# pxl-th/SLAM.jl

Hardware: AMD Instinct MI355X
Metric: frames/sec KITTI-05 stereo @1k kpts; local-BA ms/iter for 50-KF window (higher is better)
Workload: dtype f64

## Files before the change

### slam.jl_amd/csrc/common.hpp

```cpp
#pragma once
#include <hip/hip_runtime.h>
#include <cstdint>
#include <cstdio>
#include <cstring>
#include <string>
#include <vector>
#include <mutex>
#include "../../include/slamhip.h"

#define SLAM_MAX_LEVELS 8

struct slam_ctx {
    int device = 0;
    hipStream_t stream = nullptr;
    int cus = 0;
    int dev_cus = 0;
    bool arch_ok = false;
    bool xwg_ok = false;
    int pool_class = 99;
    std::string err;
    void *scratch = nullptr; size_t scratch_bytes = 0;
    void *scratch2 = nullptr; size_t scratch2_bytes = 0;
    void *pinned = nullptr; size_t pinned_bytes = 0;
    hipEvent_t wait_event = nullptr;
    hipStream_t stream2 = nullptr;
    hipEvent_t fork_ev = nullptr, join_ev = nullptr;
    bool prof_on = false;
    struct ProfSpan { int id; hipEvent_t a, b; };
    std::vector<ProfSpan> prof_pending;
    std::vector<hipEvent_t> prof_pool;
    std::vector<std::string> prof_names;
    std::vector<double> prof_ms;
    std::vector<long long> prof_cnt;
};

extern "C" hipStream_t ctx_aux_stream(slam_ctx *c);
extern "C" void ctx_probe_device(slam_ctx *c);

struct ProfScope {
    slam_ctx *c; int idx;
    ProfScope(slam_ctx *ctx, const char *name);
    ~ProfScope();
};

struct LevelView {
    double *L, *Iy, *Ix, *Iyy, *Ixx, *Iyx;
    int H, W, P;
};
struct PyrView {
    LevelView lv[SLAM_MAX_LEVELS];
    int levels;
};

struct slam_pyr {
    int device = 0;
    int levels = 0;
    int H[SLAM_MAX_LEVELS], W[SLAM_MAX_LEVELS];
    int P[SLAM_MAX_LEVELS];
    int64_t off[SLAM_MAX_LEVELS + 1];
    struct Alloc { double *base = nullptr; double *ck = nullptr; double *tot = nullptr; const void **srctab = nullptr; double *xc = nullptr; int *xf = nullptr; int xseg = 0; int refs = 0; std::mutex graph_mu; };
    Alloc *alloc = nullptr;
    size_t zstride = 0;
    int batch_index = 0, batch_size = 1;
    bool tol_planes = false;
    bool target_only = false;
    double *planes = nullptr;
    double *tmp = nullptr;
    double *ck = nullptr;
    double *norm = nullptr;
    double norm_sigma = -1.0;
    struct Graph { int mode; double sigma; int S; size_t ckmin; int src_kind; hipGraphExec_t exec; };
    std::vector<Graph> graphs;
    bool graph_failed = false;
    PyrView view;
    double *plane(int p, int l) const { return planes + (int64_t)p * off[levels] + off[l]; }
};

struct slam_kpset {
    int device = 0, S = 0, cap = 0;
    char *base = nullptr;
    double *yx = nullptr;
    double *oyx = nullptr;
    double *syx = nullptr;
    double *xyz = nullptr;
    double *kyx = nullptr;
    uint8_t *haskf = nullptr;
    double *fyx = nullptr;
    int *fkf = nullptr;
    int *kfcount = nullptr;
    int64_t *id = nullptr;
    uint8_t *is3d = nullptr, *stereo = nullptr, *st = nullptr;
    int *count = nullptr;
    int *work = nullptr;
    int *ntot = nullptr;
    int64_t *next_id = nullptr;
    double *par = nullptr, *par_host = nullptr;
    hipEvent_t par_ev[8] = {};
    int par_slot = 0;
};
int kpset_stage_params(slam_ctx *ctx, slam_kpset *ks, const double *host, size_t n, const double **dev_out);

extern thread_local std::string g_slam_err;

hipError_t slam_stream_wait(hipStream_t s);

int slam_fail(slam_ctx *ctx, int code, const char *fmt, ...);
int slam_scratch(slam_ctx *ctx, size_t bytes, void **out);
int slam_scratch2(slam_ctx *ctx, size_t bytes, void **out);
int slam_pinned(slam_ctx *ctx, size_t bytes, void **out);

#define HIP_TRY(ctx, expr)                                                                  \
    do {                                                                                    \
        hipError_t _e = (expr);                                                             \
        if (_e != hipSuccess)                                                               \
            return slam_fail((ctx), SLAM_ERR_HIP, "%s: %s (%s:%d)", #expr, hipGetErrorString(_e), __FILE__, __LINE__); \
    } while (0)

#define ARG_TRY(ctx, cond)                                                                  \
    do {                                                                                    \
        if (!(cond)) return slam_fail((ctx), SLAM_ERR_ARG, "argument check failed: %s (%s:%d)", #cond, __FILE__, __LINE__); \
    } while (0)

#define SLAM_PYR_TARGET_ONLY 16
#define SLAM_PYR_CHAIN 32
#define SLAM_PYR_FLAGS (SLAM_PYR_TARGET_ONLY | SLAM_PYR_CHAIN)
struct IIRCoef {
    double a1, a2, a3, scale, M[9], inv1masum , inv1mbsum ;
};
IIRCoef slam_iir_coef(double sigma);
int slam_gaussian_taps(double sigma, double *w);

struct Cam { double fx, fy, cx, cy; };
struct PnPArgs {
    Cam cam; const double *px; const double *pts; int n;
    double X0[6]; int iters_fast, iterations; double depth_eps, repr_eps;
    uint8_t *outl; double *result;
};
int pnp_launch_device(slam_ctx *ctx, int S, const PnPArgs *args_dev);

int kpset_build_worklist(slam_ctx *ctx, slam_kpset *ks);
int kpset_compact(slam_ctx *ctx, slam_kpset *ks, int mode, const uint8_t *flags_dev);
int slam_detect_device(slam_ctx *ctx, const double *img_dev, int H, int W, int pitch, const double *cur_yx, int n_cur,
                       int max_points, int radius, int grid_rows, int grid_cols, int cell_size,
// ... 2 lines not shown
```

### slam.jl_amd/csrc/pyramid.hip

```cpp
#include "common.hpp"
#include <cmath>
#include <cstdlib>
#include <mutex>
#include <tuple>
#include <utility>

#define LINE_THREADS 64

struct PlaneSet {
    double *p[4];
    const double *nrm[4];
    int coef[4];
    int fill0[4];
    const double *sq[4];
    int n;
    size_t zs;
};
#define PS_PICK(ps, f, pl) ((pl) == 0 ? (ps).f[0] : (pl) == 1 ? (ps).f[1] : (pl) == 2 ? (ps).f[2] : (ps).f[3])
__device__ __forceinline__ double *ps_plane(const PlaneSet &ps, int pl) { return PS_PICK(ps, p, pl) + (size_t)blockIdx.z * ps.zs; }
__device__ __forceinline__ const double *ps_nrm(const PlaneSet &ps, int pl) { return PS_PICK(ps, nrm, pl); }
__device__ __forceinline__ int ps_coef(const PlaneSet &ps, int pl) { return PS_PICK(ps, coef, pl); }
__device__ __forceinline__ bool ps_fill0(const PlaneSet &ps, int pl) { return PS_PICK(ps, fill0, pl) != 0; }
__device__ __forceinline__ const double *ps_sq(const PlaneSet &ps, int pl) { const double *q = PS_PICK(ps, sq, pl); return q ? q + (size_t)blockIdx.z * ps.zs : nullptr; }

// ... 1019 lines not shown
        const int x0 = cb * CF_W, wc = W - x0 < CF_W ? W - x0 : CF_W;
#pragma unroll
        for (int sub = 0; sub < 4; sub++)
#pragma unroll
            for (int r = 0; r < 4; r++) { const v2d t2 = {raw[sub][2 * r], raw[sub][2 * r + 1]}; *(ldsv2 *)(Cb + (8 * r + cg) * CF_LS + sub * 16 + 2 * rp) = t2; }
        cf_load_block(plane, P, cb + 1 < ncb ? x0 + CF_W : x0, r0, voff, raw);
        double acc = 0.0;
        if (SEG && w == 0 && seg > 0) {
            if (lane == 0) while (__hip_atomic_load(xf_in, __ATOMIC_RELAXED, __HIP_MEMORY_SCOPE_AGENT) <= cb) __builtin_amdgcn_s_sleep(2);
            __builtin_amdgcn_fence(__ATOMIC_ACQUIRE, "wavefront"); __builtin_amdgcn_wave_barrier();
            if (lane < CF_W && x0 + lane < W) acc = __hip_atomic_load(xc_in + x0 + lane, __ATOMIC_RELAXED, __HIP_MEMORY_SCOPE_AGENT);
        }
        if (w > 0) {
            while (flag_ld(&s_ready[w - 1]) <= cb) __builtin_amdgcn_s_sleep(1);
            __builtin_amdgcn_fence(__ATOMIC_ACQUIRE, "workgroup", "local");
            if (lane < CF_W) acc = carry_in[(cb & 1) * CF_W + lane];
            __builtin_amdgcn_fence(__ATOMIC_RELEASE, "workgroup", "local");
            if (lane == 0) flag_st(&s_done[w], cb + 1);
        }
        __builtin_amdgcn_fence(__ATOMIC_RELEASE, "wavefront"); __builtin_amdgcn_wave_barrier();
        if (lane < CF_W) {
            ldsd *c = Cb + lane * CF_LS;
            if (hr == 64 && (SEG ? r0 > 0 : w > 0)) {
#pragma unroll
                for (int half = 0; half < 2; half++) {
                    double v[32];
#pragma unroll
                    for (int j = 0; j < 16; j++) { const v2d q = *(const ldsv2 *)(c + 32 * half + 2 * j); v[2 * j] = q.x; v[2 * j + 1] = q.y; }
#pragma unroll
                    for (int e = 0; e < 32; e++) { acc = acc + v[e]; v[e] = acc; }
#pragma unroll
                    for (int j = 0; j < 16; j++) { const v2d t2 = {v[2 * j], v[2 * j + 1]}; *(ldsv2 *)(c + 32 * half + 2 * j) = t2; }
                }
            } else {
                for (int e = 0; e < hr; e++) { acc = (r0 + e == 0) ? c[e] : acc + c[e]; c[e] = acc; }
            }
        }
        if (w + 1 < nwh) {
            while (flag_ld(&s_done[w + 1]) + 2 <= cb) __builtin_amdgcn_s_sleep(1);
            if (lane < CF_W) carry_out[(cb & 1) * CF_W + lane] = acc;
            __builtin_amdgcn_fence(__ATOMIC_RELEASE, "workgroup", "local");
            if (lane == 0) flag_st(&s_ready[w], cb + 1);
        }
        else if (SEG && seg + 1 < nseg) {
            if (lane < CF_W && x0 + lane < W) __hip_atomic_store(xc_out + x0 + lane, acc, __ATOMIC_RELAXED, __HIP_MEMORY_SCOPE_AGENT);
            asm volatile("s_waitcnt vmcnt(0)" ::: "memory");
            if (lane == 0) __hip_atomic_store(xf_out, cb + 1, __ATOMIC_RELAXED, __HIP_MEMORY_SCOPE_AGENT);
        }
        __builtin_amdgcn_fence(__ATOMIC_RELEASE, "wavefront"); __builtin_amdgcn_wave_barrier();
        if (lane < hr) {
            ldsd *c = Cb + lane;
            if (wc == CF_W && cb > 0) {
                double v[CF_W];
#pragma unroll
                for (int j = 0; j < CF_W; j++) v[j] = c[j * CF_LS];
#pragma unroll
                for (int j = 0; j < CF_W; j++) { rcarry = rcarry + v[j]; v[j] = rcarry; }
#pragma unroll
                for (int j = 0; j < CF_W; j++) c[j * CF_LS] = v[j];
            } else {
                for (int j = 0; j < wc; j++) { rcarry = (cb == 0 && j == 0) ? c[j * CF_LS] : rcarry + c[j * CF_LS]; c[j * CF_LS] = rcarry; }
            }
        }
        __builtin_amdgcn_fence(__ATOMIC_RELEASE, "wavefront"); __builtin_amdgcn_wave_barrier();
#pragma unroll
        for (int sub = 0; sub < 4; sub++) {
            const int rb = r0 + sub * 16;
            if (rb < H) {
#pragma unroll
                for (int r = 0; r < 4; r++) {
                    const int col = x0 + 8 * r + cg, row = rb + 2 * rp;
                    const v2d q = *(const ldsv2 *)(Cb + (8 * r + cg) * CF_LS + sub * 16 + 2 * rp);
                    double *g = plane + ((size_t)(x0 + 8 * r) * P + rb) + voff;
                    if (col < W) {
                        if (row + 1 < H) __builtin_nontemporal_store(q, (v2d *)g);
                        else if (row < H) g[0] = q.x;
                    }
                }
            }
        }
        __builtin_amdgcn_fence(__ATOMIC_RELEASE, "wavefront"); __builtin_amdgcn_wave_barrier();
    }
    if (SEG && w == 0 && seg > 0 && lane == 0) __hip_atomic_store(xf_in, 0, __ATOMIC_RELAXED, __HIP_MEMORY_SCOPE_AGENT);
}

#define PAR_T 1024
#define PAR_SLMAX 16
#define PAR_G 8
struct SegPow { double P[2][PAR_G][9]; double Plast[2][9]; };

__device__ __forceinline__ void mv3(const double *P, double &a, double &b, double &c, double za, double zb, double zc)
{
    const double n1 = __builtin_fma(P[0], a, __builtin_fma(P[1], b, __builtin_fma(P[2], c, za)));
    const double n2 = __builtin_fma(P[3], a, __builtin_fma(P[4], b, __builtin_fma(P[5], c, zb)));
    const double n3 = __builtin_fma(P[6], a, __builtin_fma(P[7], b, __builtin_fma(P[8], c, zc)));
    a = n1; b = n2; c = n3;
}

template <int ZG, int ZL, int GG, int GL, int ZN, int GN, class Slot>
__device__ __forceinline__ void fold_entry(const SegPow &sp, int cs, double (*Z)[ZN], double (*GT)[GN],
                                           int l, int k, bool has, Slot slot, double s0a, double s0b, double s0c,
                                           double &ea, double &eb, double &ec)
{
    const int q = k % PAR_G, grp = k / PAR_G;
    const double *P1 = sp.P[cs][0], *P8 = sp.P[cs][PAR_G - 1];
    double a = 0.0, b = 0.0, c = 0.0;
    if (has) for (int i = 0; i < q; i++) { const int s = slot(grp * PAR_G + i); mv3(P1, a, b, c, Z[0][s * ZG + l * ZL], Z[1][s * ZG + l * ZL], Z[2][s * ZG + l * ZL]); }
    if (has && q == PAR_G - 1) {
        double ta = a, tb = b, tc = c; const int s = slot(k);
        mv3(P1, ta, tb, tc, Z[0][s * ZG + l * ZL], Z[1][s * ZG + l * ZL], Z[2][s * ZG + l * ZL]);
        GT[0][grp * GG + l * GL] = ta; GT[1][grp * GG + l * GL] = tb; GT[2][grp * GG + l * GL] = tc;
    }
    __syncthreads();
    double Sa = s0a, Sb = s0b, Sc = s0c;
    if (has) {
        for (int h = 0; h < grp; h++) mv3(P8, Sa, Sb, Sc, GT[0][h * GG + l * GL], GT[1][h * GG + l * GL], GT[2][h * GG + l * GL]);
        if (q > 0) mv3(sp.P[cs][q - 1], Sa, Sb, Sc, 0.0, 0.0, 0.0);
    }
    ea = Sa + a; eb = Sb + b; ec = Sc + c;
}

template <bool COLS, int T = PAR_T, int LPW = 8>
__global__ __launch_bounds__(T) void k_iir_seg(PlaneSet ps, const double *src0, int H, int W, int P, IIRPair cf, SegPow sp, int SL, int cum_mask)
{
    if (src0) src0 += (size_t)blockIdx.z * ps.zs;
    constexpr int NSEG = T / LPW, ZN = T + 8, GN = T / PAR_G + 16;
    constexpr int ZG = COLS ? 1 : LPW, ZL = COLS ? NSEG + 1 : 1, GG = COLS ? 1 : LPW, GL = COLS ? NSEG / PAR_G + 2 : 1;
    __shared__ double Z[3][ZN];
    __shared__ double GT[3][GN];
    __shared__ double Fin[3][LPW];
    const int t = threadIdx.x, l = COLS ? t / NSEG : t % LPW, g = COLS ? t % NSEG : t / LPW, pl = blockIdx.y;
    const int nlines = COLS ? W : H, n = COLS ? H : W;
    const int line = blockIdx.x * LPW + l;
    const bool valid = line < nlines;
    const int lc = valid ? line : nlines - 1;
    const long stride = COLS ? 1 : P;
    const size_t off = COLS ? (size_t)lc * P : (size_t)lc;
    double *dstp = ps_plane(ps, pl) + off;
    const double *srcp = ((pl == 0 && src0) ? src0 : ps_plane(ps, pl)) + off;
    const int cs = ps_coef(ps, pl);
    const IIRCoef &k = cf.c[cs];
    const double a1 = k.a1, a2 = k.a2, a3 = k.a3, scale = k.scale;
    const int nseg = (n + SL - 1) / SL;
    const bool has = g < nseg;
    const int b = g * SL, len = has ? min(n, b + SL) - b : 0;
    const bool lastseg = has && g == nseg - 1;
    double x[PAR_SLMAX];
#pragma unroll
    for (int j = 0; j < PAR_SLMAX; j++) x[j] = (j < len) ? srcp[(long)(b + j) * stride] : 0.0;
    const double x0 = srcp[0], xlast = srcp[(long)(n - 1) * stride];
    const double uminus = x0 / k.inv1masum;
    {
        double w1 = 0.0, w2 = 0.0, w3 = 0.0;
#pragma unroll
        for (int j = 0; j < PAR_SLMAX; j++) if (j < len) { const double tt = iir3<true>(x[j], a1, w1, a2, w2, a3, w3); w3 = w2; w2 = w1; w1 = tt; }
        if (has) { Z[0][g * ZG + l * ZL] = w1; Z[1][g * ZG + l * ZL] = w2; Z[2][g * ZG + l * ZL] = w3; }
    }
    __syncthreads();
    {
        double w1, w2, w3;
        fold_entry<ZG, ZL, GG, GL, ZN, GN>(sp, cs, Z, GT, l, g, has, [](int kk) { return kk; }, uminus, uminus, uminus, w1, w2, w3);
#pragma unroll
        for (int j = 0; j < PAR_SLMAX; j++) if (j < len) { const double tt = iir3<true>(x[j], a1, w1, a2, w2, a3, w3); w3 = w2; w2 = w1; w1 = tt; x[j] = tt; }
        if (lastseg) { Fin[0][l] = w1; Fin[1][l] = w2; Fin[2][l] = w3; }
    }
    __syncthreads();
// ... 632 lines not shown
                rq.n = 3; rq.nq0 = 0; rq.zs = zs;
                rows_tol(rq, 3, side_cum);
                return;
            }
            if (topo) {
                B.launch(k_iir_seg<false>, dim3((H + 7) / 8, 1, S), dim3(PAR_T), 0, LN_MAIN, psT, (const double *)nullptr, H, W, P, cf, spr, slr, 0);
                B.launch(k_iir_seg<false>, gr3, dim3(PAR_T), 0, side, psQ, (const double *)nullptr, H, W, P, cf, spr, slr, 0);
            }
            else if (spans) { ProfScope span(ctx, "k_iir_rows");
                B.launch(k_iir_seg<false>, gr, dim3(PAR_T), 0, LN_MAIN, ps, (const double *)nullptr, H, W, P, cf, spr, slr, 0); }
            else B.launch(k_iir_seg<false>, gr, dim3(PAR_T), 0, LN_MAIN, ps, (const double *)nullptr, H, W, P, cf, spr, slr, 0);
            if (!topo) B.fork();
            if (has_next)
                B.launch(k_resize, dim3(((size_t)p->H[l + 1] * p->W[l + 1] + 255) / 256, 1, S), dim3(256), 0, LN_MAIN,
                                   nextL, p->H[l + 1], p->W[l + 1], p->P[l + 1], (const double *)T, H, W, P, zs);
            if (c32) B.launch((k_cum_seg<true, 256, 8>), gc3, dim3(256), 0, side_cum, pc, H, W, P, slc32);
            else B.launch(k_cum_seg<true>, gc3, dim3(PAR_T), 0, side_cum, pc, H, W, P, slc);
            B.launch(k_cum_seg<false>, gr3, dim3(PAR_T), 0, side_cum, pc, H, W, P, slr);
            return;
        }
        static const bool no_tol_batch = getenv("SLAMHIP_NO_TOL_BATCH") != nullptr;
        int rt_ns = RT_NS;
        const int slr_t = rt_seg_len(W, &rt_ns);
        const bool tolb = mode == 3 && Sall >= tol_batch_min_s() && cols_fused && p->alloc->tot != nullptr && slr_t > 0 && !no_tol_batch;
        if (cols_fused) {
            ColsFusedArgs ca;
            ca.L = v.L; ca.T = has_next ? T : nullptr; ca.Iy = v.Iy; ca.Ix = v.Ix; ca.Qyy = v.Iyy; ca.Qxx = v.Ixx; ca.Qyx = v.Iyx;
            ca.H = H; ca.W = W; ca.P = P; ca.zs = zs;
            ca.src_kind = l == 0 ? src_kind : 0; ca.srctab = (const void *const *)p->alloc->srctab + z0;
            size_t toff = 0;
            for (int q = 0; q < l; q++) toff += (size_t)3 * Sall * p->W[q];
            toff += (size_t)3 * z0 * W;
            ca.tot = tolb ? p->alloc->tot + toff : nullptr; ca.tot_stride = W;
            static const bool no_dec = getenv("SLAMHIP_NO_TOL_DEC") != nullptr;
            ca.dec = (tolb && has_next && (H & 1) == 0 && (P & 31) == 0 && !no_dec) ? 1 : 0;
            if (tolb && ca.dec) B.launch(k_cols_fused<true, true>, dim3((W + CF4_COLS - 1) / CF4_COLS, 1, S), dim3(256), 0, LN_MAIN, ca, cf, p->ck);
            else if (tolb) B.launch(k_cols_fused<true, false>, dim3((W + CF4_COLS - 1) / CF4_COLS, 1, S), dim3(256), 0, LN_MAIN, ca, cf, p->ck);
            else B.launch(k_cols_fused<false, false>, dim3((W + CF4_COLS - 1) / CF4_COLS, 1, S), dim3(256), 0, LN_MAIN, ca, cf, p->ck);
            if (tolb) {
                RowsTolArgs ra = {};
                int nr = 0;
                if (has_next) { ra.p[nr] = T; ra.coef[nr] = 0; ra.kind[nr] = 0; nr++; }
                ra.nq0 = nr;
                ra.p[nr] = v.Iyy; ra.coef[nr] = 1; ra.kind[nr] = 1; nr++;
                ra.p[nr] = v.Ixx; ra.coef[nr] = 1; ra.kind[nr] = 1; nr++;
                ra.p[nr] = v.Iyx; ra.coef[nr] = 1; ra.kind[nr] = 1; nr++;
                ra.n = nr; ra.zs = zs; ra.tot = ca.tot; ra.tot_stride = W;
                const bool rzf = has_next && (H & 1) == 0;
                ra.dec = ca.dec;
                if (rzf) { ra.rz.dst = nextL; ra.rz.Hd = p->H[l + 1]; ra.rz.Wd = p->W[l + 1]; ra.rz.Pd = p->P[l + 1]; }
                SegPow spr; rt_seg_pow(cf, slr_t, spr);
                static const int rt_dbg = getenv("SLAMHIP_RT_DBG") ? atoi(getenv("SLAMHIP_RT_DBG")) : 0; ra.dbg = rt_dbg;
                const dim3 gr((H + RT_R - 1) / RT_R, nr, S), bd(RT_R * rt_ns);
                auto go = [&]() {
                    if (rt_ns != RT_NS) {
                        if (slr_t == 24) B.launch((k_rows_tol<24, 2 * RT_NS, RT_R>), gr, bd, 0, LN_MAIN, ra, H, W, P, cf, spr);
                        else B.launch((k_rows_tol<32, 2 * RT_NS, RT_R>), gr, bd, 0, LN_MAIN, ra, H, W, P, cf, spr);
                        return;
                    }
#define RT_GO(SLV) B.launch((k_rows_tol<SLV, RT_NS, RT_R>), gr, bd, 0, LN_MAIN, ra, H, W, P, cf, spr)
                    switch (slr_t) { case 4: RT_GO(4); break; case 6: RT_GO(6); break; case 8: RT_GO(8); break; case 10: RT_GO(10); break; case 12: RT_GO(12); break;
                                     case 16: RT_GO(16); break; case 20: RT_GO(20); break; case 24: RT_GO(24); break; case 32: RT_GO(32); break; default: RT_GO(40); break; }
#undef RT_GO
                };
                if (spans) { ProfScope span(ctx, "k_iir_rows"); go(); } else go();
                if (has_next && !rzf)
                    B.launch(k_resize, dim3(((size_t)p->H[l + 1] * p->W[l + 1] + 255) / 256, 1, S), dim3(256), 0, LN_MAIN,
                                       nextL, p->H[l + 1], p->W[l + 1], p->P[l + 1], (const double *)T, H, W, P, zs);
                return;
            }
        }
        else if (ck_cols) B.launch(k_iir_cols_ck, lines_grid(W, np, S), dim3(LINE_THREADS), 0, LN_MAIN, ps, src0, H, W, P, cf, p->ck);
        else if (topo) {
            B.launch(k_iir_cols<3>, lines_grid(W, 1, S), dim3(LINE_THREADS), 0, LN_MAIN, psT, src0, H, W, P, cf);
            B.launch(k_iir_cols<3>, lines_grid(W, 3, S), dim3(LINE_THREADS), 0, side, psQ, (const double *)nullptr, H, W, P, cf);
        }
        else if (S == 1) B.launch(k_iir_cols<3>, lines_grid(W, np, S), dim3(LINE_THREADS), 0, LN_MAIN, ps, src0, H, W, P, cf);
        else B.launch(k_iir_cols<2>, lines_grid(W, np, S), dim3(LINE_THREADS), 0, LN_MAIN, ps, src0, H, W, P, cf);
        const bool ck_rows = p->ck != nullptr && mode != 0 && W >= 64 && (size_t)Sall * np * H * W * 8 >= ck_min_bytes();
        static const bool no_rows_resize = getenv("SLAMHIP_NO_ROWS_RESIZE") != nullptr;
        const bool rows_resize = ck_rows && has_next && (H & 1) == 0 && !no_rows_resize;
        RowResize rz = {};
        if (rows_resize) { rz.dst = nextL; rz.Hd = p->H[l + 1]; rz.Wd = p->W[l + 1]; rz.Pd = p->P[l + 1]; }
        if (topo) {
            B.launch(k_iir_rows, lines_grid(H, 1, S), dim3(LINE_THREADS), 0, LN_MAIN, psT, H, W, P, cf);
            B.launch(k_iir_rows, lines_grid(H, 3, S), dim3(LINE_THREADS), 0, side, psQ, H, W, P, cf);
        }
        else if (spans) { ProfScope span(ctx, "k_iir_rows");
            if (ck_rows) B.launch(k_iir_rows_ck, lines_grid(H, np, S), dim3(LINE_THREADS), 0, LN_MAIN, ps, H, W, P, cf, p->ck, rz);
            else B.launch(k_iir_rows, lines_grid(H, np, S), dim3(LINE_THREADS), 0, LN_MAIN, ps, H, W, P, cf); }
        else if (ck_rows) B.launch(k_iir_rows_ck, lines_grid(H, np, S), dim3(LINE_THREADS), 0, LN_MAIN, ps, H, W, P, cf, p->ck, rz);
        else B.launch(k_iir_rows, lines_grid(H, np, S), dim3(LINE_THREADS), 0, LN_MAIN, ps, H, W, P, cf);
        if (!topo) B.fork();
        if (has_next && !rows_resize)
            B.launch(k_resize, dim3(((size_t)p->H[l + 1] * p->W[l + 1] + 255) / 256, 1, S), dim3(256), 0, LN_MAIN,
                               nextL, p->H[l + 1], p->W[l + 1], p->P[l + 1], (const double *)T, H, W, P, zs);
        static const bool no_fused_cum = getenv("SLAMHIP_NO_FUSED_CUM") != nullptr;
        const int cf_bands = (H + 63) / 64;
        const int cf_seg = cf_bands <= CF_MAXW ? 1 : (cf_bands + CF_SEGW - 1) / CF_SEGW;
        if (Sall >= 8 && !no_fused_cum && (cf_seg == 1 || (p->alloc->xc != nullptr && cf_seg <= p->alloc->xseg))) {
            const int nw = cf_seg == 1 ? cf_bands : CF_SEGW;
            const size_t lds = ((size_t)nw * CF_W * CF_LS + (size_t)nw * 2 * CF_W) * sizeof(double);
            const size_t xo = (size_t)z0 * 3 * (size_t)(cf_seg > 1 ? cf_seg - 1 : 1);
            if (cf_seg == 1) B.launch(k_cum_fused<false>, dim3(1, 3, S), dim3(nw * 64), lds, LN_AUX, pc, H, W, P, (double *)nullptr, (int *)nullptr);
            else B.launch(k_cum_fused<true>, dim3(cf_seg, 3, S), dim3(nw * 64), lds, LN_AUX, pc, H, W, P, p->alloc->xc + xo * W, p->alloc->xf + xo);
            return;
        }
        if (S == 1) B.launch(k_cum_cols<3>, lines_grid(W, 3, S), dim3(LINE_THREADS), 0, side_cum, pc, H, W, P);
        else B.launch(k_cum_cols<2>, lines_grid(W, 3, S), dim3(LINE_THREADS), 0, LN_AUX, pc, H, W, P);
        B.launch(k_cum_rows, lines_grid(H, 3, S), dim3(LINE_THREADS), 0, S == 1 ? side_cum : LN_AUX, pc, H, W, P);
    }
}


static void launch_build(slam_ctx *ctx, slam_pyr *p, int mode, const IIRPair &cf, BuildSink &B, bool spans, int S = 1, int src_kind = 0, bool target = false)
{
    bool fast = mode == 3;
    if (fast && (seg_len(p->H[0], PAR_T / 8) > PAR_SLMAX || seg_len(p->W[0], PAR_T / 8) > PAR_SLMAX)) fast = false;
    if (fast && S >= tol_batch_min_s()) fast = false;
    static const int chunk_mb = [] { const char *v = getenv("SLAMHIP_PYR_CHUNK_MB"); return v ? atoi(v) : 0; }();
    for (int l = 0; l < p->levels; l++) {
        int C = S;
        if (chunk_mb > 0 && S >= 8 && mode != 0) {
            const size_t per_image = (size_t)4 * p->P[l] * p->W[l] * 8;
            const size_t want = (size_t)chunk_mb << 20;
            if (per_image * S > 2 * want) { C = (int)std::max<size_t>(4, want / per_image); C = std::min(C, S); }
        }
        for (int z0 = 0; z0 < S; z0 += C) launch_level(ctx, p, mode, cf, B, spans, std::min(C, S - z0), src_kind, target, l, z0, S, fast);
    }
}

static bool level0_fused(const slam_pyr *p, int mode, int S)
{
    static const bool off = getenv("SLAMHIP_NO_COLS_FUSED") != nullptr || getenv("SLAMHIP_NO_SQ_FUSE") != nullptr || getenv("SLAMHIP_NO_CK_COLS") != nullptr ||
                            getenv("SLAMHIP_NO_FUSED_INGEST") != nullptr;
    if (off || mode == 0 || p->ck == nullptr || p->alloc->srctab == nullptr || p->H[0] < 64) return false;
    if (mode == 3 && S < tol_batch_min_s() && !(seg_len(p->H[0], PAR_T / 8) > PAR_SLMAX || seg_len(p->W[0], PAR_T / 8) > PAR_SLMAX)) return false;
    const int np_ = p->levels > 1 ? 4 : 3;
    return (size_t)S * np_ * p->H[0] * p->W[0] * 8 >= ck_min_bytes();
}
__global__ void k_set_ptrs(const void **tab, ImgPtrs src)
{
    if (threadIdx.x < BATCH_MAX) tab[threadIdx.x] = src.p[threadIdx.x];
}

static int enqueue_build(slam_ctx *ctx, slam_pyr *p, int mode_flags, double sigma, int S = 1, int src_kind = 0)
{
    const bool target = (mode_flags & SLAM_PYR_TARGET_ONLY) != 0;
    static const bool linear_env = getenv("SLAMHIP_LINEAR_GRAPH") != nullptr;
    const bool chain = (mode_flags & SLAM_PYR_CHAIN) != 0 || linear_env;
    const int mode = mode_flags & ~SLAM_PYR_FLAGS;
    p->target_only = target;
    p->tol_planes = mode == 3;
    if (target) src_kind |= 16;
    if (chain) src_kind |= 32;
    IIRPair cf; cf.c[0] = slam_iir_coef(sigma); cf.c[1] = slam_iir_coef(4.0);
    if (mode == 0) { int rc = build_norm(ctx, p, sigma); if (rc) return rc; }
    hipStream_t st = ctx->stream;
    static const bool no_graph = getenv("SLAMHIP_NO_GRAPH") != nullptr;
    if (ctx->prof_on || no_graph) {
        ProfScope span_all(ctx, "pyr_update");
        BuildSink B; B.st = st;
        launch_build(ctx, p, mode, cf, B, ctx->prof_on, S, src_kind & 15, target);
        HIP_TRY(ctx, hipGetLastError());
        return SLAM_OK;
    }
    hipGraphExec_t exec = nullptr;
    const size_t ckmin = ck_min_bytes();
    {
        std::lock_guard<std::mutex> lk(p->alloc->graph_mu);
        for (auto &g : p->graphs) if (g.mode == mode && g.sigma == sigma && g.S == S && g.ckmin == ckmin && g.src_kind == src_kind) exec = g.exec;
        if (!exec && !p->graph_failed) {
            hipGraph_t graph = nullptr;
            hipError_t e = hipGraphCreate(&graph, 0);
            if (e == hipSuccess) {
                BuildSink B; B.graph = graph; B.forked = !chain;
                launch_build(ctx, p, mode, cf, B, false, S, src_kind & 15, target);
                e = B.err;
            }
            if (e == hipSuccess) e = hipGraphInstantiate(&exec, graph, nullptr, nullptr, 0);
            if (graph) (void)hipGraphDestroy(graph);
            if (e != hipSuccess) { (void)hipGetLastError(); p->graph_failed = true; exec = nullptr; }
            else { slam_pyr::Graph g; g.mode = mode; g.sigma = sigma; g.S = S; g.ckmin = ckmin; g.src_kind = src_kind; g.exec = exec; p->graphs.push_back(g); }
        }
        if (exec) HIP_TRY(ctx, hipGraphLaunch(exec, st));
    }
    if (!exec) { BuildSink B; B.st = st; launch_build(ctx, p, mode, cf, B, false, S, src_kind & 15, target); }
    HIP_TRY(ctx, hipGetLastError());
    return SLAM_OK;
}

static void ingest_dense(slam_ctx *ctx, slam_pyr *p, const double *image_dev)
{
    ImgPtrs ip = {}; ip.p[0] = image_dev;
    const size_t n = (size_t)p->H[0] * p->W[0];
    hipLaunchKernelGGL(k_gather_images, dim3((n + 255) / 256, 1, 1), dim3(256), 0, ctx->stream, ip, p->plane(0, 0), p->H[0], p->W[0], p->P[0], (size_t)0);
}

extern "C" {

static int pyr_create_n(slam_ctx *ctx, int H, int W, int pyramid_levels, int S, slam_pyr **out)
{
    ARG_TRY(ctx, ctx != nullptr && out != nullptr);
    ARG_TRY(ctx, H >= 4 && W >= 4 && pyramid_levels >= 0 && pyramid_levels + 1 <= SLAM_MAX_LEVELS && S >= 1 && S <= BATCH_MAX);
    HIP_TRY(ctx, hipSetDevice(ctx->device));
    int Hs[SLAM_MAX_LEVELS], Ws[SLAM_MAX_LEVELS], Ps[SLAM_MAX_LEVELS]; int64_t off[SLAM_MAX_LEVELS + 1];
    int64_t o = 0; int h = H, w = W;
    const int levels = pyramid_levels + 1;
    for (int l = 0; l < levels; l++) {
        if (h < 4 || w < 4) return slam_fail(ctx, SLAM_ERR_ARG, "slam_pyr_create: level %d is %dx%d, too small for the IIR kernel (needs > 3)", l, h, w);
        Hs[l] = h; Ws[l] = w; Ps[l] = (h + 15) & ~15; off[l] = o; o += (int64_t)Ps[l] * w;
        h = (h + 1) / 2; w = (w + 1) / 2;
    }
    off[levels] = o;
    slam_pyr::Alloc *al = new slam_pyr::Alloc();
    const size_t tail = (size_t)64 * Ps[0];
    hipError_t e = hipMalloc((void **)&al->base, ((size_t)o * 7 * S + tail) * 8);
    if (e != hipSuccess) { delete al; return slam_fail(ctx, SLAM_ERR_HIP, "slam_pyr_create: hipMalloc: %s", hipGetErrorString(e)); }
    e = hipMemsetAsync(al->base, 0, ((size_t)o * 7 * S + tail) * 8, ctx->stream);
    if (e == hipSuccess) e = slam_stream_wait(ctx->stream);
    if (e != hipSuccess) { (void)hipFree(al->base); delete al; return slam_fail(ctx, SLAM_ERR_HIP, "slam_pyr_create: memset: %s", hipGetErrorString(e)); }
    al->refs = S;
    if (S > 1 && hipMalloc((void **)&al->srctab, BATCH_MAX * sizeof(void *)) != hipSuccess) { (void)hipGetLastError(); al->srctab = nullptr; }
    {
        hipError_t ea = hipFuncSetAttribute((const void *)k_cum_fused<false>, hipFuncAttributeMaxDynamicSharedMemorySize, 150 * 1024);
        if (ea == hipSuccess) ea = hipFuncSetAttribute((const void *)k_cum_fused<true>, hipFuncAttributeMaxDynamicSharedMemorySize, 150 * 1024);
        if (ea != hipSuccess) { (void)hipFree(al->base); delete al; return slam_fail(ctx, SLAM_ERR_HIP, "slam_pyr_create: hipFuncSetAttribute(k_cum_fused): %s", hipGetErrorString(ea)); }
    }
    double *ckbuf = nullptr;
    if (S > 1) {
        const size_t lines = (size_t)S * 4 * (((size_t)Hs[0] + LINE_THREADS - 1) / LINE_THREADS) * LINE_THREADS;
        const size_t nbk = ((size_t)Ws[0] + CK_B - 1) / CK_B;
        const size_t lines_c = (size_t)S * 4 * (((size_t)Ws[0] + CF4_COLS - 1) / CF4_COLS) * LINE_THREADS;
        const size_t nbk_c = ((size_t)Hs[0] + 31) / 32 + 1;
        const size_t need = lines * nbk > lines_c * nbk_c ? lines * nbk : lines_c * nbk_c;
        if (hipMalloc((void **)&ckbuf, need * 3 * 8) != hipSuccess) { (void)hipGetLastError(); ckbuf = nullptr; }
        al->ck = ckbuf;
        size_t wsum = 0; for (int l = 0; l < levels; l++) wsum += (size_t)Ws[l];
        if (hipMalloc((void **)&al->tot, (size_t)3 * S * wsum * 8) != hipSuccess) { (void)hipGetLastError(); al->tot = nullptr; }
        const int xbands = (Hs[0] + 63) / 64, xseg = xbands <= CF_MAXW ? 1 : (xbands + CF_SEGW - 1) / CF_SEGW;
        if (xseg > 1 && ctx->arch_ok) {
            const size_t nslot = (size_t)S * 3 * (xseg - 1);
            if (hipMalloc((void **)&al->xc, nslot * Ws[0] * 8) != hipSuccess) { (void)hipGetLastError(); al->xc = nullptr; }
            if (al->xc && (hipMalloc((void **)&al->xf, nslot * 4) != hipSuccess || hipMemset(al->xf, 0, nslot * 4) != hipSuccess)) { (void)hipGetLastError(); (void)hipFree(al->xc); al->xc = nullptr; al->xf = nullptr; }
            if (al->xc) al->xseg = xseg;
        }
    }
    for (int s = 0; s < S; s++) {
        slam_pyr *p = new slam_pyr();
        p->device = ctx->device; p->levels = levels;
        memcpy(p->H, Hs, sizeof Hs); memcpy(p->W, Ws, sizeof Ws); memcpy(p->P, Ps, sizeof Ps); memcpy(p->off, off, sizeof off);
        p->alloc = al;
        p->zstride = (size_t)o * 7;
        p->planes = al->base + (size_t)s * p->zstride;
        p->tmp = p->planes + (size_t)o * 6;
        p->batch_index = s; p->batch_size = S; p->ck = ckbuf;
        make_view(p);
        out[s] = p;
    }
    return SLAM_OK;
}

int slam_pyr_create(slam_ctx *ctx, int H, int W, int pyramid_levels, slam_pyr **out)
{
    return pyr_create_n(ctx, H, W, pyramid_levels, 1, out);
}

int slam_pyr_create_batch(slam_ctx *ctx, int H, int W, int pyramid_levels, int S, slam_pyr **out)
{
    return pyr_create_n(ctx, H, W, pyramid_levels, S, out);
}

int slam_pyr_update_batch_dev(slam_ctx *ctx, slam_pyr *const *pyrs, const double *const *images_dev, int S, int mode, double sigma, int sync)
{
    ARG_TRY(ctx, ctx != nullptr && pyrs != nullptr && images_dev != nullptr && S >= 1 && S <= BATCH_MAX && ((mode & ~SLAM_PYR_FLAGS) == 1 || (mode & ~SLAM_PYR_FLAGS) == 3) && sigma > 0);
    slam_pyr *p0 = pyrs[0];
    ARG_TRY(ctx, p0 != nullptr && p0->batch_index == 0 && p0->batch_size == S);
    for (int s = 0; s < S; s++) ARG_TRY(ctx, pyrs[s] != nullptr && pyrs[s]->alloc == p0->alloc && pyrs[s]->batch_index == s && images_dev[s] != nullptr);
    HIP_TRY(ctx, hipSetDevice(ctx->device));
    ImgPtrs ip;
    for (int s = 0; s < BATCH_MAX; s++) ip.p[s] = s < S ? images_dev[s] : nullptr;
    const size_t n = (size_t)p0->H[0] * p0->W[0];
    const bool fused_ingest = level0_fused(p0, mode & ~SLAM_PYR_FLAGS, S);
    if (fused_ingest) hipLaunchKernelGGL(k_set_ptrs, dim3(1), dim3(BATCH_MAX), 0, ctx->stream, p0->alloc->srctab, ip);
    else hipLaunchKernelGGL(k_gather_images, dim3((n + 255) / 256, 1, S), dim3(256), 0, ctx->stream, ip, p0->plane(0, 0), p0->H[0], p0->W[0], p0->P[0], p0->zstride);
    int rc = enqueue_build(ctx, p0, mode, sigma, S, fused_ingest ? 1 : 0);
    for (int s = 0; s < S; s++) { pyrs[s]->target_only = (mode & SLAM_PYR_TARGET_ONLY) != 0; pyrs[s]->tol_planes = (mode & ~SLAM_PYR_FLAGS) == 3; }
    if (rc) return rc;
    if (sync) HIP_TRY(ctx, slam_stream_wait(ctx->stream));
    return SLAM_OK;
}

int slam_pyr_update_batch_u8_dev(slam_ctx *ctx, slam_pyr *const *pyrs, const uint8_t *const *images_u8_dev, int S, int mode, double sigma, int sync)
{
    ARG_TRY(ctx, ctx != nullptr && pyrs != nullptr && images_u8_dev != nullptr && S >= 1 && S <= BATCH_MAX && ((mode & ~SLAM_PYR_FLAGS) == 1 || (mode & ~SLAM_PYR_FLAGS) == 3) && sigma > 0);
    slam_pyr *p0 = pyrs[0];
    ARG_TRY(ctx, p0 != nullptr && p0->batch_index == 0 && p0->batch_size == S);
    for (int s = 0; s < S; s++) ARG_TRY(ctx, pyrs[s] != nullptr && pyrs[s]->alloc == p0->alloc && pyrs[s]->batch_index == s && images_u8_dev[s] != nullptr);
    HIP_TRY(ctx, hipSetDevice(ctx->device));
    ImgPtrsU8 ip;
    for (int s = 0; s < BATCH_MAX; s++) ip.p[s] = s < S ? images_u8_dev[s] : nullptr;
    const size_t n = (size_t)p0->H[0] * p0->W[0];
    const bool fused_ingest = level0_fused(p0, mode & ~SLAM_PYR_FLAGS, S);
    if (fused_ingest) { ImgPtrs iq; for (int s = 0; s < BATCH_MAX; s++) iq.p[s] = (const double *)ip.p[s]; hipLaunchKernelGGL(k_set_ptrs, dim3(1), dim3(BATCH_MAX), 0, ctx->stream, p0->alloc->srctab, iq); }
    else hipLaunchKernelGGL(k_gather_images_u8, dim3((n + 255) / 256, 1, S), dim3(256), 0, ctx->stream, ip, p0->plane(0, 0), p0->H[0], p0->W[0], p0->P[0], p0->zstride);
    int rc = enqueue_build(ctx, p0, mode, sigma, S, fused_ingest ? 2 : 0);
    for (int s = 0; s < S; s++) { pyrs[s]->target_only = (mode & SLAM_PYR_TARGET_ONLY) != 0; pyrs[s]->tol_planes = (mode & ~SLAM_PYR_FLAGS) == 3; }
    if (rc) return rc;
    if (sync) HIP_TRY(ctx, slam_stream_wait(ctx->stream));
    return SLAM_OK;
}

int slam_pyr_destroy(slam_pyr *p)
{
    if (!p) return SLAM_OK;
    (void)hipSetDevice(p->device);
    (void)hipDeviceSynchronize();
    if (p->alloc && --p->alloc->refs == 0) { (void)hipFree(p->alloc->base); if (p->alloc->ck) (void)hipFree(p->alloc->ck); if (p->alloc->tot) (void)hipFree(p->alloc->tot); if (p->alloc->xc) (void)hipFree(p->alloc->xc); if (p->alloc->xf) (void)hipFree(p->alloc->xf); if (p->alloc->srctab) (void)hipFree(p->alloc->srctab); delete p->alloc; }
    if (p->norm) (void)hipFree(p->norm);
    for (auto &g : p->graphs) (void)hipGraphExecDestroy(g.exec);
    delete p;
    return SLAM_OK;
}

int slam_pyr_update_dev(slam_ctx *ctx, slam_pyr *p, const double *image_dev, int mode, double sigma, int sync)
{
    ARG_TRY(ctx, ctx != nullptr && p != nullptr && image_dev != nullptr && (mode == 0 || (mode & ~SLAM_PYR_FLAGS) == 1 || (mode & ~SLAM_PYR_FLAGS) == 3) && sigma > 0);
    HIP_TRY(ctx, hipSetDevice(ctx->device));
    ingest_dense(ctx, p, image_dev);
    int rc = enqueue_build(ctx, p, mode, sigma);
    if (rc) return rc;
    if (sync) HIP_TRY(ctx, slam_stream_wait(ctx->stream));
    return SLAM_OK;
}

int slam_pyr_update(slam_ctx *ctx, slam_pyr *p, const double *image, int mode, double sigma)
{
    ARG_TRY(ctx, ctx != nullptr && p != nullptr && image != nullptr && (mode == 0 || (mode & ~SLAM_PYR_FLAGS) == 1 || (mode & ~SLAM_PYR_FLAGS) == 3) && sigma > 0);
    HIP_TRY(ctx, hipSetDevice(ctx->device));
    void *stage;
    int rc = slam_scratch2(ctx, (size_t)p->H[0] * p->W[0] * 8, &stage);
    if (rc) return rc;
    HIP_TRY(ctx, hipMemcpyAsync(stage, image, (size_t)p->H[0] * p->W[0] * 8, hipMemcpyHostToDevice, ctx->stream));
    ingest_dense(ctx, p, (const double *)stage);
    rc = enqueue_build(ctx, p, mode, sigma);
    if (rc) return rc;
    HIP_TRY(ctx, slam_stream_wait(ctx->stream));
    return SLAM_OK;
}

int slam_pyr_update_u8(slam_ctx *ctx, slam_pyr *p, const uint8_t *image_u8, int mode, double sigma)
{
    ARG_TRY(ctx, ctx != nullptr && p != nullptr && image_u8 != nullptr && (mode == 0 || (mode & ~SLAM_PYR_FLAGS) == 1 || (mode & ~SLAM_PYR_FLAGS) == 3) && sigma > 0);
    HIP_TRY(ctx, hipSetDevice(ctx->device));
    const size_t n = (size_t)p->H[0] * p->W[0];
    void *d8;
    int rc = slam_scratch2(ctx, n, &d8);
    if (rc) return rc;
    HIP_TRY(ctx, hipMemcpyAsync(d8, image_u8, n, hipMemcpyHostToDevice, ctx->stream));
    hipLaunchKernelGGL(k_u8_to_f64, dim3((n + 255) / 256), dim3(256), 0, ctx->stream, p->plane(0, 0), (const unsigned char *)d8, p->H[0], p->W[0], p->P[0]);
    rc = enqueue_build(ctx, p, mode, sigma);
    if (rc) return rc;
    HIP_TRY(ctx, slam_stream_wait(ctx->stream));
    return SLAM_OK;
}

int slam_pyr_update_u8_dev(slam_ctx *ctx, slam_pyr *p, const uint8_t *image_u8_dev, int mode, double sigma, int sync)
{
    ARG_TRY(ctx, ctx != nullptr && p != nullptr && image_u8_dev != nullptr && (mode == 0 || (mode & ~SLAM_PYR_FLAGS) == 1 || (mode & ~SLAM_PYR_FLAGS) == 3) && sigma > 0);
    HIP_TRY(ctx, hipSetDevice(ctx->device));
    const size_t n = (size_t)p->H[0] * p->W[0];
    hipLaunchKernelGGL(k_u8_to_f64, dim3((n + 255) / 256), dim3(256), 0, ctx->stream, p->plane(0, 0), (const unsigned char *)image_u8_dev, p->H[0], p->W[0], p->P[0]);
    int rc = enqueue_build(ctx, p, mode, sigma);
    if (rc) return rc;
    if (sync) HIP_TRY(ctx, slam_stream_wait(ctx->stream));
    return SLAM_OK;
}

int slam_pyr_copy(slam_ctx *ctx, slam_pyr *dst, const slam_pyr *src)
{
    ARG_TRY(ctx, ctx != nullptr && dst != nullptr && src != nullptr);
    ARG_TRY(ctx, dst->levels == src->levels && dst->H[0] == src->H[0] && dst->W[0] == src->W[0]);
    HIP_TRY(ctx, hipSetDevice(ctx->device));
    HIP_TRY(ctx, hipMemcpyAsync(dst->planes, src->planes, (size_t)src->off[src->levels] * 6 * 8, hipMemcpyDeviceToDevice, ctx->stream));
    HIP_TRY(ctx, slam_stream_wait(ctx->stream));
    dst->target_only = src->target_only;
    dst->tol_planes = src->tol_planes;
    return SLAM_OK;
}

int slam_pyr_clone(slam_ctx *ctx, const slam_pyr *src, slam_pyr **out)
{
    ARG_TRY(ctx, ctx != nullptr && src != nullptr && out != nullptr);
    int rc = slam_pyr_create(ctx, src->H[0], src->W[0], src->levels - 1, out);
    if (rc) return rc;
    return slam_pyr_copy(ctx, *out, src);
}

int slam_pyr_shape(const slam_pyr *p, int level, int *H, int *W)
{
    if (!p || level < 0 || level >= p->levels) return SLAM_ERR_ARG;
// ... 24 lines not shown
```

Before: 22110.

## Fuse row IIR filtering with row cumulative sums into one kernel

```diff
diff --git a/slam.jl_amd/csrc/common.hpp b/slam.jl_amd/csrc/common.hpp
--- a/slam.jl_amd/csrc/common.hpp
+++ b/slam.jl_amd/csrc/common.hpp
@@ -58,7 +58,7 @@
     int H[SLAM_MAX_LEVELS], W[SLAM_MAX_LEVELS];
     int P[SLAM_MAX_LEVELS];
     int64_t off[SLAM_MAX_LEVELS + 1];
-    struct Alloc { double *base = nullptr; double *ck = nullptr; double *tot = nullptr; const void **srctab = nullptr; double *xc = nullptr; int *xf = nullptr; int xseg = 0; int refs = 0; std::mutex graph_mu; };
+    struct Alloc { double *base = nullptr; double *ck = nullptr; double *tot = nullptr; const void **srctab = nullptr; double *xc = nullptr; int *xf = nullptr; int xseg = 0; double *rck = nullptr; int refs = 0; std::mutex graph_mu; };
     Alloc *alloc = nullptr;
     size_t zstride = 0;
     int batch_index = 0, batch_size = 1;
diff --git a/slam.jl_amd/csrc/pyramid.hip b/slam.jl_amd/csrc/pyramid.hip
--- a/slam.jl_amd/csrc/pyramid.hip
+++ b/slam.jl_amd/csrc/pyramid.hip
@@ -1125,6 +1125,228 @@
         __builtin_amdgcn_fence(__ATOMIC_RELEASE, "wavefront"); __builtin_amdgcn_wave_barrier();
     }
     if (SEG && w == 0 && seg > 0 && lane == 0) __hip_atomic_store(xf_in, 0, __ATOMIC_RELAXED, __HIP_MEMORY_SCOPE_AGENT);
+}
+
+#define RC_CW 16
+#define RC_LDS_DOUBLES (RC_CW * CF_LS + 2 * RC_CW)
+__global__ __launch_bounds__(CF_MAXW * 64) void k_rows_cum(PlaneSet ps, int H, int W, int P, IIRPair cf, double *ck)
+{
+    extern __shared__ __attribute__((aligned(16))) double rc_lds[];
+    __shared__ int s_ready[CF_MAXW], s_done[CF_MAXW];
+    const int pl = blockIdx.y, lane = threadIdx.x & 63, w = threadIdx.x >> 6, nw = blockDim.x >> 6;
+    typedef __attribute__((address_space(3))) double ldsd;
+    typedef __attribute__((address_space(3))) v2d ldsv2;
+    ldsd *Cb = (ldsd *)rc_lds + (size_t)w * RC_LDS_DOUBLES;
+    ldsd *carry_out = Cb + RC_CW * CF_LS;
+    const ldsd *carry_in = carry_out - RC_LDS_DOUBLES;
+    auto flag_ld = [](int *f) { return __hip_atomic_load(f, __ATOMIC_RELAXED, __HIP_MEMORY_SCOPE_WORKGROUP); };
+    auto flag_st = [](int *f, int v) { __hip_atomic_store(f, v, __ATOMIC_RELAXED, __HIP_MEMORY_SCOPE_WORKGROUP); };
+    if (lane == 0) { flag_st(&s_ready[w], 0); flag_st(&s_done[w], 0); }
+    __syncthreads();
+    const int y = w * 64 + lane;
+    const bool live = y < H;
+    const size_t nlines = (size_t)gridDim.z * gridDim.y * blockDim.x;
+    ck += ((size_t)blockIdx.z * gridDim.y + pl) * blockDim.x;
+    const unsigned lid = threadIdx.x;
+    double *plane = ps_plane(ps, pl);
+    const unsigned yo = (unsigned)(live ? y : H - 1);
+    double *p = plane + yo;
+    const long s = P;
+    const int n = W;
+    const IIRCoef &k = ps_coef(ps, pl) == 0 ? cf.c[0] : cf.c[1];
+    const bool fill0 = ps_fill0(ps, pl);
+    const double a1 = k.a1, a2 = k.a2, a3 = k.a3, scale = k.scale;
+    const double x0 = p[0];
+    const double iminus = fill0 ? 0.0 : x0, iplus = fill0 ? 0.0 : p[(long)(n - 1) * s];
+    const double uminus = iminus / k.inv1masum;
+    const double o0 = ((x0 + a1 * uminus) + a2 * uminus) + a3 * uminus;
+    const double o1 = ((p[s] + a1 * o0) + a2 * uminus) + a3 * uminus;
+    const double o2 = ((p[2 * s] + a1 * o1) + a2 * o0) + a3 * uminus;
+    const int m = n - 6, nb = (m + CK_B - 1) / CK_B;
+    double w3 = o0, w2 = o1, w1 = o2;
+    double cur[CK_B], nxt[CK_B];
+    auto load_x = [&](int j, double *buf) {
+        const int c0 = 3 + j * CK_B, len = n - c0;
+        if (len >= CK_B) {
+#pragma unroll
+            for (int e = 0; e < CK_B; e++) buf[e] = RCK_LD(plane + (size_t)(c0 + e) * P + yo);
+        } else {
+#pragma unroll
+            for (int e = 0; e < CK_B; e++) buf[e] = e < len ? plane[(size_t)(c0 + e) * P + yo] : 0.0;
+        }
+    };
+    const int nfull = (n - 3) / CK_B, rem = (n - 3) - nfull * CK_B;
+    load_x(0, cur);
+    for (int j = 0; j < nfull; j++) {
+        load_x(j + 1, nxt);
+        if (j > 0 && j < nb) { double *c = ck + ((size_t)j * 3) * nlines + lid; CK_ST(c, w1); CK_ST(c + nlines, w2); CK_ST(c + 2 * nlines, w3); }
+#pragma unroll
+        for (int e = 0; e < CK_B; e++) { const double t = ((cur[e] + a1 * w1) + a2 * w2) + a3 * w3; w3 = w2; w2 = w1; w1 = t; }
+#pragma unroll
+        for (int e = 0; e < CK_B; e++) cur[e] = nxt[e];
+    }
+    {
+        if (nfull > 0 && nfull < nb) { double *c = ck + ((size_t)nfull * 3) * nlines + lid; CK_ST(c, w1); CK_ST(c + nlines, w2); CK_ST(c + 2 * nlines, w3); }
+#pragma unroll
+        for (int e = 0; e < CK_B; e++)
+            if (e < rem) { const double t = ((cur[e] + a1 * w1) + a2 * w2) + a3 * w3; w3 = w2; w2 = w1; w1 = t; }
+    }
+    const bool have_last = nfull == nb - 1;
+    const double uplus = iplus / k.inv1masum, vplus = uplus / k.inv1mbsum;
+    const double d0 = w1 - uplus, d1 = w2 - uplus, d2 = w3 - uplus;
+    const double vr0 = ((k.M[0] * d0 + k.M[1] * d1) + k.M[2] * d2) + vplus;
+    const double vr1 = ((k.M[3] * d0 + k.M[4] * d1) + k.M[5] * d2) + vplus;
+    const double vr2 = ((k.M[6] * d0 + k.M[7] * d1) + k.M[8] * d2) + vplus;
+    const double vA = vr0;
+    const double vB = ((w2 + a1 * vA) + a2 * vr1) + a3 * vr2;
+    const double vC = ((w3 + a1 * vB) + a2 * vA) + a3 * vr1;
+    double v1 = vC, v2 = vB, v3 = vA;
+    __builtin_amdgcn_fence(__ATOMIC_RELEASE, "workgroup"); __builtin_amdgcn_fence(__ATOMIC_ACQUIRE, "workgroup");
+    double f1n = 0, f2n = 0, f3n = 0, f1 = 0, f2 = 0, f3 = 0;
+    auto load_ck = [&](int j, double &g1, double &g2, double &g3) {
+        if (j > 0) { const double *c = ck + ((size_t)j * 3) * nlines + lid; g1 = CK_LD(c); g2 = CK_LD(c + nlines); g3 = CK_LD(c + 2 * nlines); }
+        else { g1 = o2; g2 = o1; g3 = o0; }
+    };
+    auto store_ack = [&](int j) { double *c = ck + ((size_t)j * 3) * nlines + lid; CK_ST(c, v1); CK_ST(c + nlines, v2); CK_ST(c + 2 * nlines, v3); };
+    if (nb > 1) {
+        const int j = nb - 1, len = m - j * CK_B;
+        if (!have_last) load_x(j, cur);
+        load_ck(j, f1, f2, f3);
+        load_x(j - 1, nxt); load_ck(j - 1, f1n, f2n, f3n);
+#pragma unroll
+        for (int e = 0; e < CK_B; e++)
+            if (e < len) { const double t = ((cur[e] + a1 * f1) + a2 * f2) + a3 * f3; f3 = f2; f2 = f1; f1 = t; cur[e] = t; }
+        store_ack(j);
+#pragma unroll
+        for (int e = CK_B - 1; e >= 0; e--)
+            if (e < len) { const double t = ((cur[e] + a1 * v1) + a2 * v2) + a3 * v3; v3 = v2; v2 = v1; v1 = t; }
+#pragma unroll
+        for (int e = 0; e < CK_B; e++) cur[e] = nxt[e];
+        f1 = f1n; f2 = f2n; f3 = f3n;
+    }
+    for (int j = nb - 2; j >= 1; j--) {
+        load_x(j - 1, nxt); load_ck(j - 1, f1n, f2n, f3n);
+#pragma unroll
+        for (int e = 0; e < CK_B; e++) { const double t = ((cur[e] + a1 * f1) + a2 * f2) + a3 * f3; f3 = f2; f2 = f1; f1 = t; cur[e] = t; }
+        store_ack(j);
+#pragma unroll
+        for (int e = CK_B - 1; e >= 0; e--) { const double t = ((cur[e] + a1 * v1) + a2 * v2) + a3 * v3; v3 = v2; v2 = v1; v1 = t; }
+#pragma unroll
+        for (int e = 0; e < CK_B; e++) cur[e] = nxt[e];
+        f1 = f1n; f2 = f2n; f3 = f3n;
+    }
+    if (nb > 0) store_ack(0);
+    __builtin_amdgcn_fence(__ATOMIC_RELEASE, "workgroup"); __builtin_amdgcn_fence(__ATOMIC_ACQUIRE, "workgroup");
+    double rcarry = -0.0;
+    int hk = 0;
+    auto cum_half = [&](int x0c, int wc) {
+        __builtin_amdgcn_fence(__ATOMIC_RELEASE, "wavefront"); __builtin_amdgcn_wave_barrier();
+        double acc = -0.0;
+        if (w > 0) {
+            while (flag_ld(&s_ready[w - 1]) <= hk) __builtin_amdgcn_s_sleep(1);
+            __builtin_amdgcn_fence(__ATOMIC_ACQUIRE, "workgroup", "local");
+            if (lane < RC_CW) acc = carry_in[(hk & 1) * RC_CW + lane];
+            __builtin_amdgcn_fence(__ATOMIC_RELEASE, "workgroup", "local");
+            if (lane == 0) flag_st(&s_done[w], hk + 1);
+        }
+        __builtin_amdgcn_fence(__ATOMIC_RELEASE, "wavefront"); __builtin_amdgcn_wave_barrier();
+        if (lane < wc) {
+            ldsd *c = Cb + lane * CF_LS;
+#pragma unroll
+            for (int g = 0; g < 4; g++) {
+                double v[16];
+#pragma unroll
+                for (int j = 0; j < 8; j++) { const v2d q = *(const ldsv2 *)(c + 16 * g + 2 * j); v[2 * j] = q.x; v[2 * j + 1] = q.y; }
+#pragma unroll
+                for (int e = 0; e < 16; e++) { acc = acc + v[e]; v[e] = acc; }
+#pragma unroll
+                for (int j = 0; j < 8; j++) { const v2d t2 = {v[2 * j], v[2 * j + 1]}; *(ldsv2 *)(c + 16 * g + 2 * j) = t2; }
+            }
+        }
+        if (w + 1 < nw) {
+            while (flag_ld(&s_done[w + 1]) + 2 <= hk) __builtin_amdgcn_s_sleep(1);
+            if (lane < RC_CW) carry_out[(hk & 1) * RC_CW + lane] = acc;
+            __builtin_amdgcn_fence(__ATOMIC_RELEASE, "workgroup", "local");
+            if (lane == 0) flag_st(&s_ready[w], hk + 1);
+        }
+        hk++;
+        __builtin_amdgcn_fence(__ATOMIC_RELEASE, "wavefront"); __builtin_amdgcn_wave_barrier();
+        double *q = plane + (size_t)x0c * P;
+        if (wc == RC_CW) {
+            double r[RC_CW];
+#pragma unroll
+            for (int j = 0; j < RC_CW; j++) r[j] = Cb[j * CF_LS + lane];
+#pragma unroll
+            for (int j = 0; j < RC_CW; j++) { rcarry = rcarry + r[j]; r[j] = rcarry; }
+            if (live) {
+#pragma unroll
+                for (int j = 0; j < RC_CW; j++) RCK_ST(q + (size_t)j * P + yo, r[j]);
+            }
+        } else {
+            for (int j = 0; j < wc; j++) { rcarry = rcarry + Cb[j * CF_LS + lane]; if (live) q[(size_t)j * P + yo] = rcarry; }
+        }
+        __builtin_amdgcn_fence(__ATOMIC_RELEASE, "wavefront"); __builtin_amdgcn_wave_barrier();
+    };
+    auto put = [&](int col, double v) { Cb[col * CF_LS + lane] = v; };
+    double pv0 = 0, pv1 = 0, pv2 = 0;
+    f1 = o2; f2 = o1; f3 = o0;
+    if (nb > 0) {
+        load_x(0, cur);
+        { const double *c = ck + lid; v1 = CK_LD(c); v2 = CK_LD(c + nlines); v3 = CK_LD(c + 2 * nlines); }
+    }
+    for (int j = 0; j < nb; j++) {
+        const int len = m - j * CK_B;
+        double g1n = 0, g2n = 0, g3n = 0;
+        if (len >= CK_B) {
+#pragma unroll
+            for (int e = 0; e < CK_B; e++) { const double t = ((cur[e] + a1 * f1) + a2 * f2) + a3 * f3; f3 = f2; f2 = f1; f1 = t; cur[e] = t; }
+#pragma unroll
+            for (int e = CK_B - 1; e >= 0; e--) { const double t = ((cur[e] + a1 * v1) + a2 * v2) + a3 * v3; v3 = v2; v2 = v1; v1 = t; cur[e] = t * scale; }
+        } else {
+#pragma unroll
+            for (int e = 0; e < CK_B; e++)
+                if (e < len) { const double t = ((cur[e] + a1 * f1) + a2 * f2) + a3 * f3; f3 = f2; f2 = f1; f1 = t; cur[e] = t; }
+#pragma unroll
+            for (int e = CK_B - 1; e >= 0; e--)
+                if (e < len) { const double t = ((cur[e] + a1 * v1) + a2 * v2) + a3 * v3; v3 = v2; v2 = v1; v1 = t; cur[e] = t * scale; }
+        }
+        if (j == 0) {
+            double t = ((o2 + a1 * v1) + a2 * v2) + a3 * v3; v3 = v2; v2 = v1; v1 = t; pv2 = t * scale;
+            t = ((o1 + a1 * v1) + a2 * v2) + a3 * v3; v3 = v2; v2 = v1; v1 = t; pv1 = t * scale;
+            t = ((o0 + a1 * v1) + a2 * v2) + a3 * v3; pv0 = t * scale;
+        }
+        if (j + 1 < nb) {
+            load_x(j + 1, nxt);
+            const double *c = ck + ((size_t)(j + 1) * 3) * nlines + lid; g1n = CK_LD(c); g2n = CK_LD(c + nlines); g3n = CK_LD(c + 2 * nlines);
+        }
+        const int x0 = j * CK_B;
+        if (j + 1 < nb) {
+            put(0, pv0); put(1, pv1); put(2, pv2);
+#pragma unroll
+            for (int e = 0; e < RC_CW - 3; e++) put(3 + e, cur[e]);
+            cum_half(x0, RC_CW);
+#pragma unroll
+            for (int e = RC_CW - 3; e < CK_B - 3; e++) put(e + 3 - RC_CW, cur[e]);
+            cum_half(x0 + RC_CW, RC_CW);
+            pv0 = cur[CK_B - 3]; pv1 = cur[CK_B - 2]; pv2 = cur[CK_B - 1];
+        } else {
+            const double *c = ck + ((size_t)j * 3) * nlines + lid;
+            const double t0 = CK_LD(c) * scale, t1 = CK_LD(c + nlines) * scale, t2 = CK_LD(c + 2 * nlines) * scale;
+            const int tot = len + 6;
+            for (int h = 0; h * RC_CW < tot; h++) {
+                const int lo = h * RC_CW;
+                auto putc = [&](int col, double v) { if (col >= lo && col < lo + RC_CW) put(col - lo, v); };
+                putc(0, pv0); putc(1, pv1); putc(2, pv2);
+#pragma unroll
+                for (int e = 0; e < CK_B; e++) if (e < len) putc(3 + e, cur[e]);
+                putc(len + 3, t0); putc(len + 4, t1); putc(len + 5, t2);
+                cum_half(x0 + lo, min(RC_CW, tot - lo));
+            }
+        }
+#pragma unroll
+        for (int e = 0; e < CK_B; e++) cur[e] = nxt[e];
+        v1 = g1n; v2 = g2n; v3 = g3n;
+    }
 }
 
 #define PAR_T 1024
@@ -1923,6 +2145,29 @@
         const bool rows_resize = ck_rows && has_next && (H & 1) == 0 && !no_rows_resize;
         RowResize rz = {};
         if (rows_resize) { rz.dst = nextL; rz.Hd = p->H[l + 1]; rz.Wd = p->W[l + 1]; rz.Pd = p->P[l + 1]; }
+        static const bool no_rows_cum = getenv("SLAMHIP_NO_ROWS_CUM") != nullptr;
+        static const bool no_fused_cum = getenv("SLAMHIP_NO_FUSED_CUM") != nullptr;
+        const int cf_bands = (H + 63) / 64;
+        if (!topo && Sall >= 8 && mode != 0 && W >= 64 && cf_bands <= CF_MAXW && p->alloc->rck != nullptr && !no_rows_cum && !no_fused_cum) {
+            B.fork();
+            if (has_next) {
+                PlaneSet pT = {}; pT.p[0] = ps.p[0]; pT.coef[0] = ps.coef[0]; pT.fill0[0] = ps.fill0[0]; pT.n = 1; pT.zs = zs;
+                if (spans) { ProfScope span(ctx, "k_iir_rows");
+                    if (ck_rows) B.launch(k_iir_rows_ck, lines_grid(H, 1, S), dim3(LINE_THREADS), 0, LN_MAIN, pT, H, W, P, cf, p->ck, rz);
+                    else B.launch(k_iir_rows, lines_grid(H, 1, S), dim3(LINE_THREADS), 0, LN_MAIN, pT, H, W, P, cf); }
+                else if (ck_rows) B.launch(k_iir_rows_ck, lines_grid(H, 1, S), dim3(LINE_THREADS), 0, LN_MAIN, pT, H, W, P, cf, p->ck, rz);
+                else B.launch(k_iir_rows, lines_grid(H, 1, S), dim3(LINE_THREADS), 0, LN_MAIN, pT, H, W, P, cf);
+                if (!rows_resize)
+                    B.launch(k_resize, dim3(((size_t)p->H[l + 1] * p->W[l + 1] + 255) / 256, 1, S), dim3(256), 0, LN_MAIN,
+                                       nextL, p->H[l + 1], p->W[l + 1], p->P[l + 1], (const double *)T, H, W, P, zs);
+            }
+            PlaneSet pq = {};
+            for (int q = 0; q < 3; q++) { pq.p[q] = ps.p[np - 3 + q]; pq.coef[q] = ps.coef[np - 3 + q]; pq.fill0[q] = ps.fill0[np - 3 + q]; }
+            pq.n = 3; pq.zs = zs;
+            const size_t lds = (size_t)cf_bands * RC_LDS_DOUBLES * sizeof(double);
+            B.launch(k_rows_cum, dim3(1, 3, S), dim3(cf_bands * 64), lds, LN_AUX, pq, H, W, P, cf, p->alloc->rck);
+            return;
+        }
         if (topo) {
             B.launch(k_iir_rows, lines_grid(H, 1, S), dim3(LINE_THREADS), 0, LN_MAIN, psT, H, W, P, cf);
             B.launch(k_iir_rows, lines_grid(H, 3, S), dim3(LINE_THREADS), 0, side, psQ, H, W, P, cf);
@@ -1936,8 +2181,6 @@
         if (has_next && !rows_resize)
             B.launch(k_resize, dim3(((size_t)p->H[l + 1] * p->W[l + 1] + 255) / 256, 1, S), dim3(256), 0, LN_MAIN,
                                nextL, p->H[l + 1], p->W[l + 1], p->P[l + 1], (const double *)T, H, W, P, zs);
-        static const bool no_fused_cum = getenv("SLAMHIP_NO_FUSED_CUM") != nullptr;
-        const int cf_bands = (H + 63) / 64;
         const int cf_seg = cf_bands <= CF_MAXW ? 1 : (cf_bands + CF_SEGW - 1) / CF_SEGW;
         if (Sall >= 8 && !no_fused_cum && (cf_seg == 1 || (p->alloc->xc != nullptr && cf_seg <= p->alloc->xseg))) {
             const int nw = cf_seg == 1 ? cf_bands : CF_SEGW;
@@ -2066,6 +2309,7 @@
     {
         hipError_t ea = hipFuncSetAttribute((const void *)k_cum_fused<false>, hipFuncAttributeMaxDynamicSharedMemorySize, 150 * 1024);
         if (ea == hipSuccess) ea = hipFuncSetAttribute((const void *)k_cum_fused<true>, hipFuncAttributeMaxDynamicSharedMemorySize, 150 * 1024);
+        if (ea == hipSuccess) ea = hipFuncSetAttribute((const void *)k_rows_cum, hipFuncAttributeMaxDynamicSharedMemorySize, 150 * 1024);
         if (ea != hipSuccess) { (void)hipFree(al->base); delete al; return slam_fail(ctx, SLAM_ERR_HIP, "slam_pyr_create: hipFuncSetAttribute(k_cum_fused): %s", hipGetErrorString(ea)); }
     }
     double *ckbuf = nullptr;
@@ -2077,6 +2321,10 @@
         const size_t need = lines * nbk > lines_c * nbk_c ? lines * nbk : lines_c * nbk_c;
         if (hipMalloc((void **)&ckbuf, need * 3 * 8) != hipSuccess) { (void)hipGetLastError(); ckbuf = nullptr; }
         al->ck = ckbuf;
+        if ((Hs[0] + 63) / 64 <= CF_MAXW) {
+            const size_t lines_r = (size_t)S * 3 * (((size_t)Hs[0] + 63) / 64) * 64;
+            if (hipMalloc((void **)&al->rck, lines_r * nbk * 3 * 8) != hipSuccess) { (void)hipGetLastError(); al->rck = nullptr; }
+        }
         size_t wsum = 0; for (int l = 0; l < levels; l++) wsum += (size_t)Ws[l];
         if (hipMalloc((void **)&al->tot, (size_t)3 * S * wsum * 8) != hipSuccess) { (void)hipGetLastError(); al->tot = nullptr; }
         const int xbands = (Hs[0] + 63) / 64, xseg = xbands <= CF_MAXW ? 1 : (xbands + CF_SEGW - 1) / CF_SEGW;
@@ -2157,7 +2405,7 @@
     if (!p) return SLAM_OK;
     (void)hipSetDevice(p->device);
     (void)hipDeviceSynchronize();
-    if (p->alloc && --p->alloc->refs == 0) { (void)hipFree(p->alloc->base); if (p->alloc->ck) (void)hipFree(p->alloc->ck); if (p->alloc->tot) (void)hipFree(p->alloc->tot); if (p->alloc->xc) (void)hipFree(p->alloc->xc); if (p->alloc->xf) (void)hipFree(p->alloc->xf); if (p->alloc->srctab) (void)hipFree(p->alloc->srctab); delete p->alloc; }
+    if (p->alloc && --p->alloc->refs == 0) { (void)hipFree(p->alloc->base); if (p->alloc->ck) (void)hipFree(p->alloc->ck); if (p->alloc->tot) (void)hipFree(p->alloc->tot); if (p->alloc->xc) (void)hipFree(p->alloc->xc); if (p->alloc->xf) (void)hipFree(p->alloc->xf); if (p->alloc->rck) (void)hipFree(p->alloc->rck); if (p->alloc->srctab) (void)hipFree(p->alloc->srctab); delete p->alloc; }
     if (p->norm) (void)hipFree(p->norm);
     for (auto &g : p->graphs) (void)hipGraphExecDestroy(g.exec);
     delete p;
```

Result: faster. 23450 (median of 6 runs) (+6.0%).
